# jpfuentes2/swim

Measured on NVIDIA B200. Metric: simulated node-rounds/sec, higher is better.
Workload: dtype u8/u32

## Files before the change

swim_b200/csrc/swim_device.cuh:

```cuda
#pragma once
#include <cuda_runtime.h>
#include <stdint.h>

#include "../../include/swim.h"

#ifdef SWIM_EMU
#define SWIM_LAUNCH(kernel, grid, block, stream, ...) swim_emu::launch((grid), (block), [=] { kernel(__VA_ARGS__); })
#define SWIM_SHARED_1D(T, name, n) static char name##_tag; T *name = (T *)swim_emu::shared(&name##_tag, sizeof(T) * (n))
#define SWIM_SHARED_2D(T, name, n0, n1) static char name##_tag; T (*name)[n1] = (T (*)[n1])swim_emu::shared(&name##_tag, sizeof(T) * (n0) * (n1))
#else
#define SWIM_LAUNCH(kernel, grid, block, stream, ...) kernel<<<(grid), (block), 0, (stream)>>>(__VA_ARGS__)
#define SWIM_SHARED_1D(T, name, n) __shared__ T name[n]
#define SWIM_SHARED_2D(T, name, n0, n1) __shared__ T name[n0][n1]
#endif

namespace swim {

struct DevEvent;

#ifndef SWIM_WARPS_PER_BLOCK
#define SWIM_WARPS_PER_BLOCK 8
#endif
constexpr int kWarpsPerBlock = SWIM_WARPS_PER_BLOCK;
constexpr int kMinBlocks = 32 / kWarpsPerBlock;
// ... 1354 lines not shown
  if (batching && warp == 0 && lane == 0) d.qm[0] = 0;
  for (uint32_t it = 0; it < d.nrounds; ++it) {
    const uint32_t round = d.round + it;
    tl_mark(d, round, 0);
    if (warp == 0 && lane == 0) { d.wl_cnt[ci(round + 1)] = 0; d.ncand[ci(round + 1)] = 0; }
    if (batching && prev_quiet && d.nrounds - it >= 2) {
      const uint32_t Q = d.qbatch < d.nrounds - it ? d.qbatch : d.nrounds - it;
      if (warp == 0 && lane == 0) d.qm[(nb + 1) % 3] = 0;
      uint32_t p1 = 0;
      uint32_t busy = quiet_scan<W>(d, round, Q, warp, nwarps, lane, p1);
      busy = __reduce_or_sync(kFull, busy);
      if (lane == 0 && busy) atomicOr(&d.qm[nb % 3], busy);
      tl_mark(d, round, 1);
      grid_barrier(d, round, 5);
      const uint32_t mask = *(volatile uint32_t *)&d.qm[nb % 3];
      ++nb;
      const uint32_t fb = mask ? (uint32_t)__ffs(mask) - 1u : Q;
      tl_mark(d, round, 2);
      tl_mark(d, round, 7, fb);
      c.v[SWIM_CTR_PINGS] += p1 * fb;
      prev_quiet = fb == Q;
      if (fb) { it += fb - 1; continue; }
    }
    const uint32_t *skip = nullptr;
    if (mail) {
      recv_pass<W>(d, round - 1, warp, nwarps, lane, pbs, c, round);
      skip = d.mailbits + (size_t)((round - 1) % 3u) * d.mbw;
    }
    uint32_t pings = 0;
    scan_pass<W>(d, round, warp, nwarps, lane, pings, skip, pbs.s);
    c.v[SWIM_CTR_PINGS] += pings;
    tl_mark(d, round, 1);
    const uint32_t *wl_cnt_r = d.wl_cnt + ci(round);
    if (sharded) grid_barrier_leader(d, false, round, [&] { return *(volatile const uint32_t *)wl_cnt_r == 0; }, 5);
    else grid_barrier(d, round, 5);
    tl_mark(d, round, 2);
    const uint32_t n_work = d.wl_cnt[ci(round)];
    const uint32_t first_ln = first_work_entry(d, round, warp);
    if (mail) {
      uint32_t *mb = d.mailbits + (size_t)((round - 1) % 3u) * d.mbw;
      for (uint32_t x = warp * 32 + lane; x < d.mbw; x += nwarps * 32) mb[x] = 0;
    }
    prev_quiet = n_work == 0 && !mail;
    if (n_work) {
      const bool remote = work_pass<W>(d, round, warp, nwarps, lane, pbs, c, first_ln, false);
      tl_mark(d, round, 3);
      if (sharded) grid_barrier_leader(d, cta_or(remote), round, [] { return true; }, 6);
      else grid_barrier(d, round, 6);
      tl_mark(d, round, 4);
    }
    uint32_t got = n_work ? *(volatile uint32_t *)&d.ncand[ci(round)] : 0u;
    if (sharded)
      for (uint32_t a = 0; a < d.world; ++a)
        if (a != d.rank) got |= *(volatile uint32_t *)&d.rcnt[(round & 1) * d.world + a];
    mail = got != 0;
    if (mail) prev_quiet = false;
  }
  if (mail) {
    recv_pass<W>(d, d.round + d.nrounds - 1, warp, nwarps, lane, pbs, c, 0);
    uint32_t *mb = d.mailbits + (size_t)((d.round + d.nrounds - 1) % 3u) * d.mbw;
    for (uint32_t x = warp * 32 + lane; x < d.mbw; x += nwarps * 32) mb[x] = 0;
  }
  c.flush(d.ctr, lane);
}


template <int W>
__device__ __forceinline__ void tick_decide(const SimDev &d, uint32_t tick_round, uint32_t ln, const Row<W> &row, uint32_t pbcnt,
                                            const uint32_t (&td)[W], int lane, Ctr &c, uint32_t *listbits) {
  const uint32_t self = d.first + ln;
  uint32_t am[W], sus = 0, L = 0, risk = d.loss_ppm;
#pragma unroll
  for (int w = 0; w < W; ++w) {
    am[w] = __ballot_sync(kFull, (row.st[w] & 3u) == SWIM_ALIVE);
    sus |= __ballot_sync(kFull, (row.st[w] & 3u) == SWIM_SUSPECT);
    L += __popc(am[w]);
    risk |= am[w] & td[w];
  }
  bool need = pbcnt != 0 || sus != 0;
  if (L && risk && !need) {
    const uint4 x = target_block<W>(d, tick_round, self >> 2);
    uint32_t ldraw = 0;
    if (d.loss_ppm) ldraw = word_of(philox4x32_10(make_uint4(tick_round, self >> 2, P_LOSS0, 0), d.key0, d.key1), self & 3);
    need = probe_fails<W>(d, am, td, L, word_of(x, self & 3), ldraw, tick_round, self);
  }
  if (lane == 0) {
    if (L) c.v[SWIM_CTR_PINGS] += d.P < L ? d.P : L;
    if (need) {
      wl_of(d, tick_round)[atomicAdd(&d.wl_cnt[ci(tick_round)], 1u)] = ln;
      if (listbits) atomicOr(&listbits[ln >> 5], 1u << (ln & 31));
    }
  }
}

template <int W>
__device__ __forceinline__ void x_node(const SimDev &d, uint32_t round, uint32_t ln, uint32_t idx, bool from_wl, bool mail, bool early,
                                       uint32_t snd, int lane, PbStage &pbs, Ctr &c, bool decide, bool &did_remote,
                                       uint32_t next_ln, bool have_next) {
  const uint32_t mround = round - 1, mpar = mround & 1;
  uint32_t old = 0, wbit = 0, mbit = 0;
  if (!from_wl) {
    if (lane == 0) old = atomicExch(&d.claim[ln], mround);
    wbit = d.workbits[(size_t)(round % 3u) * d.mbw + (ln >> 5)] >> (ln & 31) & 1u;
  } else if (mail) {
    mbit = d.mailbits[(size_t)(mround % 3u) * d.mbw + (ln >> 5)] >> (ln & 31) & 1u;
  }
  Row<W> row;
  row_load<W>(row, d, ln, lane);
  pb_load(pbs, d, ln, lane);
  uint32_t rix[W], td[W];
#pragma unroll
  for (int w = 0; w < W; ++w) {
    rix[w] = W <= 2 ? d.ridx[(size_t)ln * d.cap + w * 32 + lane] : 0u;
    td[w] = d.meta[(size_t)ln * W + w].z;
  }
  uint32_t e0 = 0, e1 = 0, self_inc = 0;
  uint4 early_rec = make_uint4(0, 0, 0, 0);
  uint32_t early_cnt = 0;
  if (!from_wl || mail) {
    e0 = d.in_off[ln]; e1 = d.in_off[ln + 1];
    self_inc = d.self_inc[ln];
    if (early) {
      if ((uint32_t)lane < d.B) early_rec = d.out[((size_t)mpar * d.per + snd) * d.B + lane];
      early_cnt = d.out_cnt[(size_t)mpar * d.per + snd];
    }
  }
  if (!from_wl) {
    if (wbit || __shfl_sync(kFull, old, 0) == mround) return;
  }
  const bool has_mail = !from_wl || mbit != 0;
  bool do_work = from_wl;
  if (has_mail) {
    uint32_t l_pre = 0;
#pragma unroll
    for (int w = 0; w < W; ++w) l_pre += __popc(__ballot_sync(kFull, (row.st[w] & 3u) == SWIM_ALIVE));
    const uint32_t self_inc0 = self_inc;
    apply_mail<W>(d, mround, ln, e0, e1, early, snd, early_rec, early_cnt, row, pbs, self_inc, lane, c);
    row_store<W>(row, d, ln, lane, mround);
    row.touched = 0;
    row.ticked = 0;
    if (lane == 0 && self_inc != self_inc0) d.self_inc[ln] = self_inc;
    uint32_t am[W], sus = 0, l_post = 0, risk = d.loss_ppm;
#pragma unroll
    for (int w = 0; w < W; ++w) {
      am[w] = __ballot_sync(kFull, (row.st[w] & 3u) == SWIM_ALIVE);
      sus |= __ballot_sync(kFull, (row.st[w] & 3u) == SWIM_SUSPECT);
      l_post += __popc(am[w]);
      risk |= am[w] & td[w];
    }
    const uint32_t p_pre = d.P < l_pre ? d.P : l_pre, p_post = d.P < l_post ? d.P : l_post;
    if (lane == 0) c.v[SWIM_CTR_PINGS] += p_post - p_pre;
    if (!from_wl) {
      do_work = pbs.cnt != 0 || sus != 0;
      if (l_post && risk && !do_work) {
        const uint32_t self = d.first + ln;
        const uint4 x = target_block<W>(d, round, self >> 2);
        uint32_t ldraw = 0;
        if (d.loss_ppm) ldraw = word_of(philox4x32_10(make_uint4(round, self >> 2, P_LOSS0, 0), d.key0, d.key1), self & 3);
        do_work = probe_fails<W>(d, am, td, l_post, word_of(x, self & 3), ldraw, round, self);
      }
      if (do_work) {
        if (lane == 0) {
          idx = atomicAdd(&d.wl_cnt[ci(round)], 1u);
          wl_of(d, round)[idx] = ln;
        }
        idx = __shfl_sync(kFull, idx, 0);
      }
    }
  }
  if (do_work) work_body<W>(d, round, ln, idx, row, rix, td, pbs, c, lane, did_remote, next_ln, have_next);
  else pb_store(pbs, d, ln, lane);
  if (decide) tick_decide<W>(d, round + 1, ln, row, pbs.cnt, td, lane, c, d.workbits + (size_t)((round + 1) % 3u) * d.mbw);
}

__device__ __forceinline__ void grid_barrier_freeze(const SimDev &d, const uint32_t *cnt_src, uint32_t *cnt_dst, uint32_t tl_round, int tl_slot) {
  __syncthreads();
  if (threadIdx.x == 0) {
    volatile uint32_t *gen = d.gbar + 1;
    const uint32_t g = (*barrier_generation())++;
    __threadfence();
    if (atomicAdd(d.gbar, 1u) == gridDim.x - 1) {
      __threadfence();
      tl_mark_last(d, tl_round, tl_slot);
      *(volatile uint32_t *)cnt_dst = *(volatile const uint32_t *)cnt_src;
      d.gbar[0] = 0;
      __threadfence();
      atomicAdd(d.gbar + 1, 1u);
    } else {
      const long long t0 = clock64();
      uint32_t polls = 0;
      while (*gen == g) {
        if (wait_expired(d, t0, 6000000000ll, polls, 2)) break;
        __nanosleep(20);
      }
    }
    __threadfence();
  }
  __syncthreads();
}

__device__ __forceinline__ void grid_barrier_leader_freeze(const SimDev &d, bool fence_sys, uint32_t mail_round, const uint32_t *cnt_src,
                                                           uint32_t *cnt_dst, int tl_slot) {
  SWIM_SHARED_1D(uint32_t, s_last, 1);
  __syncthreads();
  if (threadIdx.x == 0) {
    if (fence_sys) __threadfence_system(); else __threadfence();
    const bool last = atomicAdd(d.gbar, 1u) == gridDim.x - 1;
    if (last) { __threadfence(); tl_mark_last(d, mail_round, tl_slot); }
    s_last[0] = last ? 1u : 0u;
  }
  __syncthreads();
  if (s_last[0]) {
    peer_handshake_cta(d, mail_round);
    __syncthreads();
    if (threadIdx.x == 0) {
      (*barrier_generation())++;
      *(volatile uint32_t *)cnt_dst = *(volatile const uint32_t *)cnt_src;
      d.gbar[0] = 0;
      __threadfence();
      atomicAdd(d.gbar + 1, 1u);
    }
  } else if (threadIdx.x == 0) {
    volatile uint32_t *gen = d.gbar + 1;
    const uint32_t g = (*barrier_generation())++;
    const long long t0 = clock64();
    uint32_t polls = 0;
    while (*gen == g) {
      if (wait_expired(d, t0, kPeerWaitCycles + 6000000000ll, polls, 2)) break;
      __nanosleep(20);
    }
    __threadfence();
  }
  __syncthreads();
}

template <int W>
__global__ void __launch_bounds__(kThreads, kMinBlocks) round_kernel_x(SimDev d) {
  SWIM_SHARED_2D(uint4, s_pb, kWarpsPerBlock, 32);
  const int lane = threadIdx.x & 31, wib = threadIdx.x >> 5;
  const uint32_t warp = blockIdx.x * kWarpsPerBlock + wib, nwarps = gridDim.x * kWarpsPerBlock;
  pdl_launch();
  pdl_wait();
  barrier_begin(d);
  Ctr c; c.clear();
  PbStage pbs; pbs.s = s_pb[wib];
  const bool batching = d.qbatch > 1 && d.world == 1 && d.loss_ppm == 0;
  const bool sharded = d.world > 1 && d.p2p;
  const uint32_t last_round = d.round + d.nrounds - 1;
  bool mail = false;
  bool have_wl = false;
  bool known_empty = false;
  bool wb_prev = false;
  bool mail_prev = false;
  uint32_t nb = 0;
  if (batching && warp == 0 && lane == 0) d.qm[0] = 0;
  for (uint32_t it = 0; it < d.nrounds; ++it) {
    const uint32_t round = d.round + it;
    if (!have_wl) {
      if (warp == 0 && lane == 0) { d.wl_cnt[ci(round + 1)] = 0; d.ncand[ci(round)] = 0; }
      uint32_t pings = 0;
      scan_pass<W>(d, round, warp, nwarps, lane, pings, nullptr, pbs.s, nullptr, d.workbits + (size_t)(round % 3u) * d.mbw);
      c.v[SWIM_CTR_PINGS] += pings;
      grid_barrier_freeze(d, d.wl_cnt + ci(round), d.wl_n + ci(round), round, -1);
      have_wl = true;
      known_empty = false;
    }
    tl_mark(d, round, 0);
    const uint32_t n_work = known_empty ? 0u : *(volatile const uint32_t *)&d.wl_n[ci(round)];
    const bool last = round == last_round;
    if (wb_prev) {
      uint32_t *wb = d.workbits + (size_t)((round - 1) % 3u) * d.mbw;
      for (uint32_t x = warp * 32 + lane; x < d.mbw; x += nwarps * 32) wb[x] = 0;
    }
    if (mail_prev) {
      uint32_t *mb = d.mailbits + (size_t)((round - 2) % 3u) * d.mbw;
      for (uint32_t x = warp * 32 + lane; x < d.mbw; x += nwarps * 32) mb[x] = 0;
    }
    if (batching && n_work == 0 && !mail && !last) {
      const uint32_t Q = d.qbatch < last_round - round ? d.qbatch : last_round - round;
      if (warp == 0 && lane == 0) {
        d.qm[(nb + 1) % 3] = 0;
        d.wl_cnt[ci(round + 1)] = 0; d.wl_cnt[ci(round + 2)] = 0; d.ncand[ci(round + 1)] = 0;
      }
      uint32_t p1 = 0;
      uint32_t busy = quiet_scan<W>(d, round + 1, Q, warp, nwarps, lane, p1);
      busy = __reduce_or_sync(kFull, busy);
      if (lane == 0 && busy) atomicOr(&d.qm[nb % 3], busy);
      tl_mark(d, round, 1);
      grid_barrier(d, round, 5);
      const uint32_t mask = *(volatile uint32_t *)&d.qm[nb % 3];
      ++nb;
      const uint32_t fb = mask ? (uint32_t)__ffs(mask) - 1u : Q;
      tl_mark(d, round, 2);
      tl_mark(d, round, 7, fb == Q ? Q : fb + 1);
      c.v[SWIM_CTR_PINGS] += p1 * fb;
      if (fb == Q) { it += Q - 1; known_empty = true; }
      else { it += fb; have_wl = false; known_empty = false; }
      wb_prev = false;
      mail_prev = false;
      continue;
    }
    if (warp == 0 && lane == 0) { d.wl_cnt[ci(round + 2)] = 0; d.ncand[ci(round + 1)] = 0; }
    bool did_remote = false;
    if (mail) {
      const uint32_t mpar = (round - 1) & 1;
      const uint32_t w0 = nwarps - 1 - warp;
      const uint32_t n_cl = d.ncand[ci(round - 1)];
      const uint2 *cl_in = d.cl + (size_t)mpar * d.n * d.fanout;
      for (uint32_t item = w0; item < n_cl; item += nwarps) {
        const uint2 e = cl_in[item];
        x_node<W>(d, round, e.x, 0u, false, true, true, e.y, lane, pbs, c, !last, did_remote, 0u, false);
      }
      if (d.world > 1) {
        uint32_t seg_end[SWIM_MAX_WORLD + 1];
        uint32_t n_recv = 0;
        seg_end[0] = 0;
        for (uint32_t a = 0; a < d.world; ++a) {
          if (a != d.rank) n_recv += d.rcnt[mpar * d.world + a];
          seg_end[1 + a] = n_recv;
        }
        for (uint32_t item = w0; item < n_recv; item += nwarps) {
          uint32_t a = 0;
          while (item >= seg_end[1 + a]) ++a;
          const uint32_t ln = d.rlr[((size_t)mpar * d.world + a) * d.rcap + (item - seg_end[a])];
          x_node<W>(d, round, ln, 0u, false, true, false, 0u, lane, pbs, c, !last, did_remote, 0u, false);
        }
      }
    }
    if (n_work) {
      const uint32_t *wl = wl_of(d, round);
      uint32_t next_ln = warp < n_work ? *(volatile const uint32_t *)(wl + warp) : 0u;
      for (uint32_t idx = warp; idx < n_work; idx += nwarps) {
        const uint32_t ln = next_ln;
        const bool have_next = idx + nwarps < n_work;
        if (have_next) next_ln = *(volatile const uint32_t *)(wl + idx + nwarps);
        x_node<W>(d, round, ln, idx, true, mail, false, 0u, lane, pbs, c, !last, did_remote, next_ln, have_next);
      }
    }
    if (!last) {
      uint32_t pings = 0;
      scan_pass<W>(d, round + 1, warp, nwarps, lane, pings, mail ? d.mailbits + (size_t)((round - 1) % 3u) * d.mbw : nullptr, pbs.s,
                   n_work ? d.workbits + (size_t)(round % 3u) * d.mbw : nullptr, d.workbits + (size_t)((round + 1) % 3u) * d.mbw);
      c.v[SWIM_CTR_PINGS] += pings;
    }
    tl_mark(d, round, 1);
    if (sharded) grid_barrier_leader_freeze(d, cta_or(did_remote), round, d.wl_cnt + ci(round + 1), d.wl_n + ci(round + 1), 5);
    else grid_barrier_freeze(d, d.wl_cnt + ci(round + 1), d.wl_n + ci(round + 1), round, 5);
    tl_mark(d, round, 2);
    tl_mark(d, round, 4, (unsigned long long)(n_work || mail));
    mail_prev = mail;
    wb_prev = n_work != 0;
    uint32_t got = *(volatile uint32_t *)&d.ncand[ci(round)];
    if (sharded)
      for (uint32_t a = 0; a < d.world; ++a)
        if (a != d.rank) got |= *(volatile uint32_t *)&d.rcnt[(round & 1) * d.world + a];
    mail = got != 0;
    known_empty = false;
  }
  if (mail) recv_pass<W>(d, last_round, warp, nwarps, lane, pbs, c, 0);
  for (uint32_t x = warp * 32 + lane; x < d.mbw; x += nwarps * 32) {
    d.mailbits[(size_t)(last_round % 3u) * d.mbw + x] = 0;
    d.mailbits[(size_t)((last_round + 2u) % 3u) * d.mbw + x] = 0;
    d.workbits[x] = 0; d.workbits[d.mbw + x] = 0; d.workbits[2 * (size_t)d.mbw + x] = 0;
  }
  c.flush(d.ctr, lane);
}

__device__ __forceinline__ void mark_observers(const SimDev &d, uint32_t node, bool crashed, int lane) {
  const uint32_t W = d.cap >> 5;
  for (uint32_t x = d.obs_off[node] + lane, end = d.obs_off[node + 1]; x < end; x += 32) {
    const uint32_t slot = d.obs_slot[x], l = slot / d.cap, s = slot % d.cap;
    uint32_t *word = reinterpret_cast<uint32_t *>(d.meta + (size_t)l * W + (s >> 5)) + 2;
    if (crashed) atomicOr(word, 1u << (s & 31)); else atomicAnd(word, ~(1u << (s & 31)));
  }
}

static __global__ void __launch_bounds__(kThreads) derive_meta_kernel(SimDev d) {
  const int lane = threadIdx.x & 31;
  const uint32_t warp = (blockIdx.x * blockDim.x + threadIdx.x) >> 5, nwarps = (gridDim.x * blockDim.x) >> 5;
  const uint32_t W = d.cap >> 5;
  for (uint32_t l = warp; l < d.n; l += nwarps)
    for (uint32_t w = 0; w < W; ++w) {
      const size_t x = (size_t)l * d.cap + w * 32 + lane;
      const uint32_t live = d.vst[x] & 3u;
      const unsigned am = __ballot_sync(kFull, live == SWIM_ALIVE);
      const unsigned sm = __ballot_sync(kFull, live == SWIM_SUSPECT);
      const unsigned td = __ballot_sync(kFull, live != SWIM_VACANT && d.alive[d.nbr[x]] == 0);
      if (lane == 0) {
        const uint32_t flags = w == 0 ? (d.alive[d.first + l] ? 1u : 0u) | ((uint32_t)d.pb_cnt[l] << 8) : 0u;
        d.meta[(size_t)l * W + w] = make_uint4(am, sm, td, flags);
      }
    }
}

struct DevEvent {
  uint32_t node;
  uint32_t kind;
  uint4 rec;
};

static __global__ void __launch_bounds__(256) churn_kernel(SimDev d) {
  pdl_launch();
  pdl_wait();
  const uint32_t round = d.round;
  uint32_t *const cnt = d.churn_cnt + (round & 1u);
  if (blockIdx.x == 0 && threadIdx.x == 0) d.churn_cnt[(round + 1u) & 1u] = 0;
  for (uint32_t g = blockIdx.x * blockDim.x + threadIdx.x; 4 * g < d.N; g += gridDim.x * blockDim.x) {
    const uint32_t base = 4 * g;
    uint32_t up4 = 0;
    if (base + 4 <= d.N) up4 = *reinterpret_cast<const uint32_t *>(d.alive + base);
    else for (uint32_t j = 0; base + j < d.N; ++j) up4 |= (uint32_t)d.alive[base + j] << (8 * j);
    const uint4 x = philox4x32_10(make_uint4(round, g, P_CHURN, 0), d.key0, d.key1);
    uint4 y = make_uint4(0, 0, 0, 0);
    bool have_y = false;
#pragma unroll
    for (int j = 0; j < 4; ++j) {
      const uint32_t i = base + j;
      if (i >= d.N) break;
      uint32_t kind = 0xFFFFFFFFu;
      if (up4 >> (8 * j) & 0xFFu) {
        if (bounded(word_of(x, j), 1000000u) < d.churn_ppm) {
          if (!have_y) { y = philox4x32_10(make_uint4(round, g, P_CHURN, 1), d.key0, d.key1); have_y = true; }
          d.back_at[i] = round + d.rejoin_min + bounded(word_of(y, j), d.rejoin_span);
          kind = SWIM_EV_CRASH;
        }
      } else if (d.back_at[i] == round) {
        d.back_at[i] = 0;
        kind = SWIM_EV_REJOIN;
      }
      if (kind != 0xFFFFFFFFu) {
        const uint32_t k = atomicAdd(cnt, 1u);
        if (k < d.churn_cap) { d.churn_ev[k].node = i; d.churn_ev[k].kind = kind; d.churn_ev[k].rec = make_uint4(0, 0, 0, 0); }
        else *d.bar_err = 3;
      }
    }
  }
}

template <int W>
__global__ void __launch_bounds__(kThreads) event_kernel(SimDev d, const DevEvent *ev, uint32_t n_ev, const uint32_t *n_ev_dev) {
  SWIM_SHARED_2D(uint4, s_pb, kWarpsPerBlock, 32);
  const int lane = threadIdx.x & 31, wib = threadIdx.x >> 5;
  const uint32_t warp = blockIdx.x * kWarpsPerBlock + wib, nwarps = gridDim.x * kWarpsPerBlock;
  pdl_launch();
  pdl_wait();
  Ctr c; c.clear();
  PbStage pbs; pbs.s = s_pb[wib];
  const uint32_t round = d.round;
  if (n_ev_dev) n_ev = *n_ev_dev < d.churn_cap ? *n_ev_dev : d.churn_cap;
  for (uint32_t x0 = warp; x0 < n_ev; x0 += nwarps) {
   const uint32_t node = ev[x0].node;
   if (x0 && ev[x0 - 1].node == node) continue;
   for (uint32_t x = x0; x < n_ev && ev[x].node == node; ++x) {
    const uint32_t kind = ev[x].kind;
    const bool local = node >= d.first && node < d.first + d.n;
    const uint32_t ln = node - d.first;
    if (kind == SWIM_EV_CRASH) {
      const bool was_up = d.alive[node] != 0;
      __syncwarp();
      if (lane == 0) {
        d.alive[node] = 0;
        if (was_up) d.last_crash[node] = round;
        if (local) reinterpret_cast<uint8_t *>(d.meta + (size_t)ln * (d.cap >> 5))[12] = 0;
      }
      mark_observers(d, node, true, lane);
    } else if (kind == SWIM_EV_REJOIN) {
      const bool was_up = d.alive[node] != 0;
      __syncwarp();
      if (!was_up) {
        if (lane == 0) {
          d.alive[node] = 1;
          d.last_rejoin[node] = round;
          if (local) reinterpret_cast<uint8_t *>(d.meta + (size_t)ln * (d.cap >> 5))[12] = 1;
        }
        mark_observers(d, node, false, lane);
        if (local) {
          uint32_t inc = d.self_inc[ln] + 1;
          __syncwarp();
          if (lane == 0) d.self_inc[ln] = inc;
          pb_load(pbs, d, ln, lane);
          pb_enqueue(pbs, d, make_rec(node, inc, 0, SWIM_MSG_ALIVE), lane, c.v[SWIM_CTR_PB_DROPPED]);
          pb_store(pbs, d, ln, lane);
        }
      }
    } else if (local && d.alive[node] != 0) {
      Row<W> row;
      row_load<W>(row, d, ln, lane);
      pb_load(pbs, d, ln, lane);
      uint32_t self_inc = d.self_inc[ln];
      const uint32_t self_inc0 = self_inc;
      uint4 rb;
      if (row_apply<W>(row, d, node, self_inc, ev[x].rec, rb, lane, c.v[SWIM_CTR_REFUTES]) == 1) {
        pb_enqueue(pbs, d, rb, lane, c.v[SWIM_CTR_PB_DROPPED]);
        if (lane == 0) ++c.v[SWIM_CTR_RECS_APPLIED];
      }
      row_store<W>(row, d, ln, lane, round);
      pb_store(pbs, d, ln, lane);
      if (lane == 0 && self_inc != self_inc0) d.self_inc[ln] = self_inc;
    }
    __syncwarp();
   }
  }
  c.flush(d.ctr, lane);
}

__device__ __forceinline__ uint64_t fmix64(uint64_t x) {
  x ^= x >> 33; x *= 0xff51afd7ed558ccdull; x ^= x >> 33; x *= 0xc4ceb9fe1a85ec53ull; x ^= x >> 33;
  return x;
}
__device__ __forceinline__ uint64_t dg3(uint64_t tag, uint64_t idx, uint64_t w0, uint64_t w1) {
  return fmix64(fmix64(fmix64(idx + (tag << 56)) ^ w0) ^ w1);
}

static __global__ void __launch_bounds__(kThreads) digest_kernel(SimDev d, unsigned long long *out) {
  const size_t tid = (size_t)blockIdx.x * blockDim.x + threadIdx.x, nthr = (size_t)gridDim.x * blockDim.x;
  uint64_t acc = 0;
  const size_t slots = (size_t)d.n * d.cap;
  for (size_t x = tid; x < slots; x += nthr) {
    const uint64_t gi = (uint64_t)d.first * d.cap + x;
    acc += dg3(2, gi, (uint64_t)d.nbr[x] | ((uint64_t)d.vinc[x] << 32), (uint64_t)d.vst[x] | ((uint64_t)d.vlast[x] << 8));
  }
  for (size_t l = tid; l < d.n; l += nthr) {
    const uint64_t g = d.first + l;
    acc += dg3(1, g, (uint64_t)d.self_inc[l] | ((uint64_t)d.seqno[l] << 32), (uint64_t)d.alive[g] | ((uint64_t)d.pb_cnt[l] << 8));
  }
  const size_t recs = (size_t)d.n * d.B;
  for (size_t x = tid; x < recs; x += nthr) {
    const size_t l = x / d.B, q = x % d.B;
    if (q >= d.pb_cnt[l]) continue;
    const uint4 r = d.pb[x];
    acc += dg3(3, (uint64_t)d.first * d.B + x, (uint64_t)r.x | ((uint64_t)r.y << 32),
               (uint64_t)r.z | ((uint64_t)(r.w & 0xFFu) << 32) | ((uint64_t)((r.w >> 8) & 0xFFu) << 40));
  }
#pragma unroll
  for (int o = 16; o; o >>= 1) acc += __shfl_xor_sync(kFull, acc, o);
  if ((threadIdx.x & 31) == 0 && acc) atomicAdd(out, (unsigned long long)acc);
}

__device__ __forceinline__ uint32_t count_mismatches(const SimDev &d) {
  const uint32_t W = d.cap >> 5;
  uint32_t bad = 0;
  for (size_t l = (size_t)blockIdx.x * blockDim.x + threadIdx.x; l < d.n; l += (size_t)gridDim.x * blockDim.x) {
    const uint4 m0 = d.meta[l * W];
    if ((m0.w & 0xFFu) == 0) continue;
    for (uint32_t w = 0; w < W; ++w) {
      const uint4 m = w ? d.meta[l * W + w] : m0;
      bad += __popc(m.z & (m.x | m.y)) + __popc(m.y & ~m.z);
      uint32_t rest = ~(m.x | m.y | m.z);
      while (rest) {
        const uint32_t s = __ffs(rest) - 1;
        rest &= rest - 1;
        bad += (d.vst[l * d.cap + w * 32 + s] & 3u) == SWIM_DEAD;
      }
    }
  }
  return bad;
}

static __global__ void __launch_bounds__(kThreads) mismatch_kernel(SimDev d, unsigned long long *out) {
  const uint32_t bad = __reduce_add_sync(kFull, count_mismatches(d));
  if ((threadIdx.x & 31) == 0 && bad) atomicAdd(out, (unsigned long long)bad);
}

static __global__ void __launch_bounds__(kThreads) observe_kernel(SimDev d, unsigned long long *acc, uint32_t *done,
                                                                  volatile unsigned long long *host_out, unsigned long long seq) {
  SWIM_SHARED_1D(uint32_t, s_last, 1);
  pdl_launch();
  pdl_wait();
  const uint32_t bad = __reduce_add_sync(kFull, count_mismatches(d));
  if ((threadIdx.x & 31) == 0 && bad) atomicAdd(acc, (unsigned long long)bad);
  __threadfence();
  __syncthreads();
  if (threadIdx.x == 0) {
    s_last[0] = atomicAdd(done, 1u) == gridDim.x - 1 ? 1u : 0u;
    __threadfence();
  }
  __syncthreads();
  if (!s_last[0]) return;
  if (threadIdx.x < SWIM_CTR__COUNT) host_out[threadIdx.x] = *(volatile unsigned long long *)&d.ctr[threadIdx.x];
  if (threadIdx.x == 0) {
    host_out[SWIM_CTR__COUNT] = atomicExch(acc, 0ull);
    host_out[SWIM_CTR__COUNT + 1] = *(volatile uint32_t *)d.bar_err;
    *done = 0;
  }
  __threadfence_system();
  __syncthreads();
  if (threadIdx.x == 0) host_out[SWIM_CTR__COUNT + 2] = seq;
}

}
```

Before: 45.02 billion.

## Merge mail and worklist jobs into one interleaved warp job stream

New measurement: 44.94 billion (median of 6 runs). Within noise of the previous version (-0.2%).

```diff
diff --git a/swim_b200/csrc/swim_device.cuh b/swim_b200/csrc/swim_device.cuh
--- a/swim_b200/csrc/swim_device.cuh
+++ b/swim_b200/csrc/swim_device.cuh
@@ -1680,44 +1680,52 @@
     }
     if (warp == 0 && lane == 0) { d.wl_cnt[ci(round + 2)] = 0; d.ncand[ci(round + 1)] = 0; }
     bool did_remote = false;
+#ifndef SWIM_XJOB_INTERLEAVE
+#define SWIM_XJOB_INTERLEAVE 1
+#endif
+#ifndef SWIM_XSCAN_TOPDOWN
+#define SWIM_XSCAN_TOPDOWN 1
+#endif
+    const uint32_t jw = SWIM_XJOB_INTERLEAVE ? wib * gridDim.x + blockIdx.x : warp;
+    uint32_t j = jw, n_rx = 0;
     if (mail) {
       const uint32_t mpar = (round - 1) & 1;
-      const uint32_t w0 = nwarps - 1 - warp;
       const uint32_t n_cl = d.ncand[ci(round - 1)];
       const uint2 *cl_in = d.cl + (size_t)mpar * d.n * d.fanout;
-      for (uint32_t item = w0; item < n_cl; item += nwarps) {
-        const uint2 e = cl_in[item];
+      for (; j < n_cl; j += nwarps) {
+        const uint2 e = cl_in[j];
         x_node<W>(d, round, e.x, 0u, false, true, true, e.y, lane, pbs, c, !last, did_remote, 0u, false);
       }
+      n_rx = n_cl;
       if (d.world > 1) {
         uint32_t seg_end[SWIM_MAX_WORLD + 1];
-        uint32_t n_recv = 0;
-        seg_end[0] = 0;
+        seg_end[0] = n_cl;
         for (uint32_t a = 0; a < d.world; ++a) {
-          if (a != d.rank) n_recv += d.rcnt[mpar * d.world + a];
-          seg_end[1 + a] = n_recv;
-        }
-        for (uint32_t item = w0; item < n_recv; item += nwarps) {
+          if (a != d.rank) n_rx += d.rcnt[mpar * d.world + a];
+          seg_end[1 + a] = n_rx;
+        }
+        for (; j < n_rx; j += nwarps) {
           uint32_t a = 0;
-          while (item >= seg_end[1 + a]) ++a;
-          const uint32_t ln = d.rlr[((size_t)mpar * d.world + a) * d.rcap + (item - seg_end[a])];
+          while (j >= seg_end[1 + a]) ++a;
+          const uint32_t ln = d.rlr[((size_t)mpar * d.world + a) * d.rcap + (j - seg_end[a])];
           x_node<W>(d, round, ln, 0u, false, true, false, 0u, lane, pbs, c, !last, did_remote, 0u, false);
         }
       }
     }
     if (n_work) {
-      const uint32_t *wl = wl_of(d, round);
-      uint32_t next_ln = warp < n_work ? *(volatile const uint32_t *)(wl + warp) : 0u;
-      for (uint32_t idx = warp; idx < n_work; idx += nwarps) {
+      const uint32_t *wl = wl_of(d, round) - n_rx;
+      const uint32_t n_jobs = n_rx + n_work;
+      uint32_t next_ln = j < n_jobs ? *(volatile const uint32_t *)(wl + j) : 0u;
+      for (; j < n_jobs; j += nwarps) {
         const uint32_t ln = next_ln;
-        const bool have_next = idx + nwarps < n_work;
-        if (have_next) next_ln = *(volatile const uint32_t *)(wl + idx + nwarps);
-        x_node<W>(d, round, ln, idx, true, mail, false, 0u, lane, pbs, c, !last, did_remote, next_ln, have_next);
+        const bool have_next = j + nwarps < n_jobs;
+        if (have_next) next_ln = *(volatile const uint32_t *)(wl + j + nwarps);
+        x_node<W>(d, round, ln, j - n_rx, true, mail, false, 0u, lane, pbs, c, !last, did_remote, next_ln, have_next);
       }
     }
     if (!last) {
       uint32_t pings = 0;
-      scan_pass<W>(d, round + 1, warp, nwarps, lane, pings, mail ? d.mailbits + (size_t)((round - 1) % 3u) * d.mbw : nullptr, pbs.s,
+      scan_pass<W>(d, round + 1, SWIM_XSCAN_TOPDOWN ? nwarps - 1 - jw : warp, nwarps, lane, pings, mail ? d.mailbits + (size_t)((round - 1) % 3u) * d.mbw : nullptr, pbs.s,
                    n_work ? d.workbits + (size_t)(round % 3u) * d.mbw : nullptr, d.workbits + (size_t)((round + 1) % 3u) * d.mbw);
       c.v[SWIM_CTR_PINGS] += pings;
     }
```
